# Banus/pano360

Hardware: AMD Instinct MI355X
Metric: blended megapixels/sec (multiband) (higher is better)
Workload: dtype f32; 1 GPU; cfg3: 32 synthetic 3840x2160 frames per image set, spherical warp + multiband blend L=5, native resolution (MAX_RESOLUTION uncapped); frames=32

## Files before the change

### include/pano360.h

```cpp
#ifndef PANO360_H
#define PANO360_H

#include <stddef.h>
#include <stdint.h>

#ifdef __cplusplus
extern "C" {
#endif

#define PANO_OK 0
#define PANO_EINVAL (-1)
#define PANO_EHIP (-2)
#define PANO_ELIMIT (-3)
#define PANO_ESOLVE (-4)

#define PANO_MAX_TAPS 129
#define PANO_MAX_LEVELS 8
#define PANO_TAP_LEAD 7
#define PANO_TAP_PAD 40
#ifndef PANO_INTERIOR_BLOCK
#define PANO_INTERIOR_BLOCK 4
#endif
#ifndef PANO_MEDIAN_KEEP
#define PANO_MEDIAN_KEEP 32
// ... 46 lines not shown


const char *pano_version(void);
const char *pano_last_error(void);
int pano_device_count(void);
int pano_pitch(int w);
int pano_interior_block(void);

typedef struct pano_ctx pano_ctx;
#define PANO_OPT_BLUR_KERNEL 0
#define PANO_OPT_OWN_PRUNE 1
#define PANO_OPT_BLUR_SEGMENTS 2
#define PANO_OPT_BLUR_LEAN 3
#define PANO_OPT_STITCH_STREAMS 4
#define PANO_OPT_STITCH_ASYNC 5
#define PANO_OPT_BLUR_SEG_LEN 6
#define PANO_OPT_SIFT_GRAPH 7
#define PANO_OPT_LEVEL_CLASSES 8
#define PANO_OPT_COUNT 9
#define PANO_BLUR_MFMA 0
#define PANO_BLUR_VALU 1
int pano_ctx_create(int device, void *stream, pano_ctx **out);
int pano_ctx_destroy(pano_ctx *ctx);
int pano_ctx_set_stream(pano_ctx *ctx, void *stream);
int pano_ctx_set_option(pano_ctx *ctx, int option, int value);
int pano_ctx_get_option(const pano_ctx *ctx, int option, int *value);

int pano_timing_enable(pano_ctx *ctx, int on);
int pano_kernel_count(void);
const char *pano_kernel_name(int kid);
int pano_timing_read(pano_ctx *ctx, int kid, double *total_ms, int *launches);

int pano_add_weights(pano_ctx *ctx, const uint8_t *frame, int h, int w,
                     const float *lut255, const double *hat_x, const double *hat_y,
                     float *rgba);

int pano_warp_spherical(pano_ctx *ctx, const uint8_t *frame, int sh, int sw,
                        const double *proj, const double *sin_t, const double *cos_t,
                        const double *tan_p, const float *lut255, const double *hat_x,
                        const double *hat_y, int gx0, int gy0, int pw, int ph,
                        float *planes, uint8_t *mask, float *map_x, float *map_y);

int pano_warp_windows(pano_ctx *ctx, const pano_camera *cams, const pano_patch *patches,
                      int n, int max_vw, int max_vh, const double *sin_t,
                      const double *cos_t, const double *tan_p, const float *lut,
                      int lut_stride, const uint8_t *need);

int pano_ownership(pano_ctx *ctx, const pano_patch *patches, int n, int H, int W,
                   int16_t *owner, uint8_t *valid);

int pano_ownership_cameras(pano_ctx *ctx, const pano_camera *cams, int n, int H, int W,
                           int xs0, int xs1, const double *sin_t, const double *cos_t,
                           const double *tan_p, int16_t *owner, uint8_t *valid);

int pano_owned_regions(pano_ctx *ctx, const int16_t *owner, int H, int W, int xs0, int xs1,
                       int n, int min_gap, int max_spans, uint8_t *marks,
                       int32_t *regions);

int pano_ownership_regions(pano_ctx *ctx, const pano_camera *cams, int n, int H, int W,
                           int xs0, int xs1, const double *sin_t, const double *cos_t,
                           const double *tan_p, int16_t *owner, uint8_t *valid,
                           int min_gap, int max_spans, uint8_t *marks, int32_t *regions);

int pano_blur_tile_grid(const pano_ctx *ctx);
int pano_blur_tiles(pano_ctx *ctx, const pano_patch *patches, int n, int max_aw,
                    int max_ah, int W, int radius, const uint8_t *interior,
                    uint8_t *tile_flags, uint8_t *warp_need);
int pano_multiband_blur_prepare(pano_ctx *ctx, const pano_patch *patches, int n,
                                int max_aw, int max_ah, int W, const uint8_t *interior,
                                uint8_t *tile_flags);
int pano_multiband_blur(pano_ctx *ctx, const pano_patch *patches, int n, int max_aw,
                        int max_vh, int max_ah, const int16_t *owner, int W,
                        const float *taps, const int *ntaps, int n_blur,
                        const uint8_t *interior, uint8_t *tile_flags);

int pano_interior_map(pano_ctx *ctx, const int16_t *owner, int H, int W, int xs0, int xs1,
                      int radius, int16_t *block_owner, uint8_t *interior);
int pano_interior_classes(pano_ctx *ctx, const int16_t *owner, int H, int W, int xs0, int xs1,
                          const int *radii, int n_radii, int16_t *block_owner, uint8_t *interior,
                          uint8_t *classes);

int pano_layout_windows(int tile_grid, const int32_t *regions, int n, int max_spans,
                        const int32_t *rects, const uint8_t *have, int radius,
                        int xs0, int xs1, int n_blur, pano_patch *records, int cap,
                        pano_layout *out);
int pano_layout_place(pano_patch *records, int n_records, void *planes, void *blurred,
                      void *scratch);

int pano_multiband_compose(pano_ctx *ctx, const pano_patch *patches, int n, int H, int W,
                           int xs0, int xs1, int n_levels, const int16_t *owner,
                           const uint8_t *valid, const uint8_t *interior,
                           const uint8_t *classes, const pano_camera *cams,
                           const double *sin_t, const double *cos_t, const double *tan_p,
                           const float *lut, int lut_stride, uint8_t *mosaic,
                           float *mosaic_f32);

int pano_blend_cameras(pano_ctx *ctx, const pano_camera *cams, int n, int H, int W,
                       int xs0, int xs1, int linear, const double *sin_t,
                       const double *cos_t, const double *tan_p, const float *lut,
                       int lut_stride, uint8_t *mosaic, uint8_t *valid);

int pano_median_cameras(pano_ctx *ctx, const pano_camera *cams, int n, int H, int W,
                        int xs0, int xs1, float tol, const double *sin_t,
                        const double *cos_t, const double *tan_p, const float *lut,
                        int lut_stride, uint8_t *mosaic, uint8_t *valid);

// ... 321 lines not shown
```

### pano360_amd/_lib.py

```python
import ctypes as C
import os
import subprocess

_HERE = os.path.dirname(os.path.abspath(__file__))
LIB_PATH = os.environ.get("PANO_LIB") or os.path.join(_HERE, "libpano360_hip.so")

MAX_TAPS = 129
MAX_LEVELS = 8
TAP_LEAD = 7
TAP_PAD = 40
OPT_BLUR_KERNEL, OPT_OWN_PRUNE, OPT_BLUR_SEGMENTS, OPT_BLUR_LEAN, OPT_STITCH_STREAMS = 0, 1, 2, 3, 4
OPT_STITCH_ASYNC = 5
OPT_BLUR_SEG_LEN = 6
OPT_SIFT_GRAPH = 7
OPT_LEVEL_CLASSES = 8
BLUR_MFMA, BLUR_VALU = 0, 1


class PanoError(RuntimeError):
    """A C-ABI call returned a negative status."""


class Patch(C.Structure):
    _fields_ = [("planes", C.c_void_p), ("mask", C.c_void_p),
# ... 86 lines not shown
class PhotoFrame(C.Structure):
    _fields_ = [("img", C.c_void_p), ("pitch", C.c_int64), ("w", C.c_int32), ("h", C.c_int32)]


class PhotoPair(C.Structure):
    _fields_ = [("H", C.c_double * 9), ("i", C.c_int32), ("j", C.c_int32)]


class PhotoApply(C.Structure):
    _fields_ = [("src", C.c_void_p), ("dst", C.c_void_p), ("table", C.c_void_p),
                ("src_pitch", C.c_int64), ("dst_pitch", C.c_int64),
                ("w", C.c_int32), ("h", C.c_int32)]


class Pair(C.Structure):
    _fields_ = [("minv", C.c_double * 9), ("i", C.c_int32), ("j", C.c_int32)]


class SiftKeypoint(C.Structure):
    _fields_ = [("x", C.c_float), ("y", C.c_float), ("size", C.c_float), ("angle", C.c_float),
                ("response", C.c_float), ("octave", C.c_int32), ("r", C.c_int32), ("c", C.c_int32)]


class Camera(C.Structure):
    _fields_ = [("proj", C.c_double * 9), ("frame", C.c_void_p),
                ("hat_x", C.c_void_p), ("hat_y", C.c_void_p),
                ("sh", C.c_int32), ("sw", C.c_int32),
                ("y0", C.c_int32), ("x0", C.c_int32), ("h", C.c_int32), ("w", C.c_int32)]


_vp, _i = C.c_void_p, C.c_int
_SIGNATURES = {
    "pano_version": (C.c_char_p, []),
    "pano_last_error": (C.c_char_p, []),
    "pano_device_count": (_i, []),
    "pano_pitch": (_i, [_i]),
    "pano_interior_block": (_i, []),
    "pano_ctx_create": (_i, [_i, _vp, C.POINTER(C.c_void_p)]),
    "pano_ctx_destroy": (_i, [_vp]),
    "pano_ctx_set_stream": (_i, [_vp, _vp]),
    "pano_ctx_set_option": (_i, [_vp, _i, _i]),
    "pano_ctx_get_option": (_i, [_vp, _i, C.POINTER(C.c_int)]),
    "pano_timing_enable": (_i, [_vp, _i]),
    "pano_kernel_count": (_i, []),
    "pano_kernel_name": (C.c_char_p, [_i]),
    "pano_timing_read": (_i, [_vp, _i, C.POINTER(C.c_double), C.POINTER(C.c_int)]),
    "pano_add_weights": (_i, [_vp, _vp, _i, _i, _vp, _vp, _vp, _vp]),
    "pano_warp_spherical": (_i, [_vp, _vp, _i, _i, _vp, _vp, _vp, _vp, _vp, _vp, _vp, _i, _i, _i,
                                 _i, _vp, _vp, _vp, _vp]),
    "pano_warp_windows": (_i, [_vp, _vp, _vp, _i, _i, _i, _vp, _vp, _vp, _vp, _i, _vp]),
    "pano_blur_tiles": (_i, [_vp, _vp, _i, _i, _i, _i, _i, _vp, _vp, _vp]),
    "pano_ownership": (_i, [_vp, _vp, _i, _i, _i, _vp, _vp]),
    "pano_ownership_cameras": (_i, [_vp, _vp, _i, _i, _i, _i, _i, _vp, _vp, _vp, _vp, _vp]),
    "pano_owned_regions": (_i, [_vp, _vp, _i, _i, _i, _i, _i, _i, _i, _vp, _vp]),
    "pano_ownership_regions": (_i, [_vp, _vp, _i, _i, _i, _i, _i, _vp, _vp, _vp, _vp, _vp,
                                    _i, _i, _vp, _vp]),
    "pano_multiband_blur": (_i, [_vp, _vp, _i, _i, _i, _i, _vp, _i, _vp, C.POINTER(C.c_int), _i,
                                 _vp, _vp]),
    "pano_multiband_blur_prepare": (_i, [_vp, _vp, _i, _i, _i, _i, _vp, _vp]),
    "pano_layout_windows": (_i, [_i, _vp, _i, _i, _vp, _vp, _i, _i, _i, _i, _vp, _i, _vp]),
    "pano_layout_place": (_i, [_vp, _i, _vp, _vp, _vp]),
    "pano_interior_map": (_i, [_vp, _vp, _i, _i, _i, _i, _i, _vp, _vp]),
    "pano_interior_classes": (_i, [_vp, _vp, _i, _i, _i, _i, _vp, _i, _vp, _vp, _vp]),
    "pano_multiband_compose": (_i, [_vp, _vp, _i, _i, _i, _i, _i, _i, _vp, _vp, _vp, _vp, _vp, _vp,
                                    _vp, _vp, _vp, _i, _vp, _vp]),
    "pano_blend_cameras": (_i, [_vp, _vp, _i, _i, _i, _i, _i, _i, _vp, _vp, _vp, _vp, _i, _vp,
                                _vp]),
    "pano_blur_tile_grid": (_i, [_vp]),
    "pano_overlap_blocks": (_i, [_i, _i]),
    "pano_overlap_stats": (_i, [_vp, _vp, _vp, _i, _i, _i, _i, _vp, _vp, _vp]),
    "pano_linear_blend": (_i, [_vp, _vp, _i, _i, _i, _vp]),
    "pano_no_blend": (_i, [_vp, _vp, _i, _i, _i, _vp]),
    "pano_median_cameras": (_i, [_vp, _vp, _i, _i, _i, _i, _i, C.c_float, _vp, _vp, _vp, _vp, _i,
                                 _vp, _vp]),
    "pano_median_blend": (_i, [_vp, _vp, _i, _i, _i, C.c_float, _vp]),
    "pano_crop_rect": (_i, [_vp, _vp, _i, _i, _vp, _vp]),
    "pano_blur_plane": (_i, [_vp, _vp, _vp, _vp, _i, _i, _i, _vp, _i]),
    "pano_pyr_down": (_i, [_vp, _vp, _i, _i, _vp]),
    "pano_gray_u8": (_i, [_vp, _vp, _i, _i, _vp]),
    "pano_scale_step": (_i, [_vp, _vp, _i, _i, _vp, _i, _vp, _vp]),
    "pano_scale_space": (_i, [_vp, _vp, _i, _i, _i, _i, _vp, _vp, _vp, _vp, _vp]),
    "pano_resize_up2": (_i, [_vp, _vp, _i, _i, _vp]),
    "pano_decimate2": (_i, [_vp, _vp, _i, _i, _vp]),
    "pano_subtract": (_i, [_vp, _vp, _vp, C.c_size_t, _vp]),
    "pano_pyr_down_image": (_i, [_vp, _vp, _i, _i, _i, _i, _vp]),
    "pano_pyr_up_image": (_i, [_vp, _vp, _i, _i, _i, _i, _vp, _i, _vp, _i, _i]),
    "pano_u8_to_f32": (_i, [_vp, _vp, C.c_size_t, _vp]),
    "pano_laplacian_mix": (_i, [_vp, _vp, _vp, _vp, C.c_size_t, _i, _vp]),
    "pano_clip_u8": (_i, [_vp, _vp, C.c_size_t, _i, _vp]),
    "pano_poisson_blend": (_i, [_vp, _vp, _vp, _vp, _i, _i, _i, C.c_double, _i, _vp, _vp, _vp]),
    "pano_seam_levels": (_i, [_vp, _vp, _vp, _i, _i, _i, _i, _i, _vp, _vp]),
    "pano_seam_flood": (_i, [_vp, _vp, _i, _i, _i, _i, _vp, _vp]),
    "pano_seam_mask": (_i, [_vp, _vp, _i, _i, _vp, _vp, _vp, _i, _i]),
    "pano_alpha_blend": (_i, [_vp, _vp, _vp, _i, _vp, _i, C.c_int64, C.c_int64, C.c_int64, _i, _i,
                              _i, _vp]),
    "pano_resize_u8": (_i, [_vp, _vp, _i, _i, _i, _vp, _vp, _vp, _i, _i]),
    "pano_sift_extrema": (_i, [_vp, _vp, _i, _i, _i, _i, C.c_float, C.c_float, C.c_float, _vp,
                               _vp, _i]),
    "pano_sift_orient": (_i, [_vp, _vp, _vp, _i, _vp, _vp, _i, _vp, _vp, _i]),
    "pano_sift_describe": (_i, [_vp, _vp, _vp, _i, _vp, _i, _vp, _vp]),
    "pano_sift_sort_work_bytes": (C.c_size_t, [_i]),
    "pano_sift_sort_unique": (_i, [_vp, _vp, _i, _vp, _i, _vp, _vp, _vp]),
    "pano_knn2_work_bytes": (C.c_size_t, [_i, _i, _i]),
    "pano_knn2": (_i, [_vp, _vp, _i, _vp, _i, _i, C.c_float, _vp, _vp, _vp, _vp]),
    "pano_hom_ransac_work_bytes": (C.c_size_t, [_i, _i]),
    "pano_hom_ransac": (_i, [_vp, _vp, _vp, _vp, _i, _i, C.c_float, C.c_uint64, _vp, _vp, _vp, _vp,
# ... 134 lines not shown
```

### pano360_amd/csrc/blend.hip

```cpp
#include <stdlib.h>

#include "geom.h"

__global__ __launch_bounds__(256) void ownership_kernel(
    const pano_patch *__restrict__ patches, int n, int H, int W,
    int16_t *__restrict__ owner, uint8_t *__restrict__ valid) {
    const int x = blockIdx.x * 64 + threadIdx.x, y = blockIdx.y * 4 + threadIdx.y;
    if (x >= W || y >= H) return;
    float best = 0.0f;
    int who = -1;
    bool any = false;
    for (int i = 0; i < n; ++i) {
        const pano_patch p = patches[i];
        const int px = x - p.x0, py = y - p.y0;
        if ((unsigned)px >= (unsigned)p.w || (unsigned)py >= (unsigned)p.h) continue;
        const float a = p.planes[3 * (size_t)p.vh * p.vpitch + (size_t)py * p.vpitch + px];
        if (a > best) {
            best = a;
            who = i;
        }
        any |= p.mask[(size_t)py * p.w + px] == 0;
    }
    owner[(size_t)y * W + x] = (int16_t)who;
    valid[(size_t)y * W + x] = any ? 1 : 0;
// ... 355 lines not shown
#pragma unroll 1
        for (int y = sy0 + wave; y < sy1; y += 4) {
            const double t = tan_p[y];
            float best = 0.0f;
            int who = -1, who_k = 0;
            bool any = false;
            for (int k = 0; k < ncand; ++k) {
                const int i = listed < 0 ? k : __builtin_amdgcn_readfirstlane(list[k]);
                const pano_camera *cam = cams + i;
                const int px = xc - cam->x0, py = y - cam->y0;
                if ((unsigned)px >= (unsigned)cam->w || (unsigned)py >= (unsigned)cam->h) continue;
                float fx, fy;
                const int sw = cam->sw, sh_ = cam->sh;
                if (map_pixel(cam->proj, s, c, t, sw, sh_, fx, fy)) continue;
                any = true;
                const Taps tp = make_taps_unmasked(fx, fy, sw, sh_);
                const float a = alpha_at(cam->hat_x, cam->hat_y, tp);
                if (a > best) {
                    best = a;
                    who = i;
                    who_k = k;
                }
            }
            if (in_strip) {
                owner[(size_t)y * W + x] = (int16_t)who;
                valid[(size_t)y * W + x] = any ? 1 : 0;
            }
            if (marks) {
                if (who != run_o) {
                    flush();
                    run_o = who;
                    run_pos = pruned && who >= 0 ? s_pos[sub][who_k] : who_k;
                    run_y0 = y;
                }
                run_y1 = y;
            }
        }
    }
    if (!marks) return;
    flush();
    __syncthreads();
    const int tid = wave * 64 + lane;
    if (tid < listed) {
        const int *b = s_box[tid];
        if (b[1] >= b[0]) box_merge(boxes + (size_t)box_stride * sh.list[tid], b[0], b[1], b[2], b[3]);
    }
}

#define OW_T 64
#define OW_Q 16
#define OW_CAMS 32
#define OW_QLIST 8
#define OW_ILP 4
#define OW_EVAL (-3)
#define OW_NOBODY (-1)
#define OW_UNOWNED (-2)

#define OW_SUBS 8
#define OW_FN(name) name
#include "own_tile.inc"
#undef OW_FN
#define OW_TH_TALL (OW_Q * OW_SUBS)

template <bool LINEAR, bool PERCAM>
__global__ __launch_bounds__(256) void blend_cameras_kernel(
    const pano_camera *__restrict__ cams, int n, int H, int W, int xs0, int xs1,
    const double *__restrict__ sin_t, const double *__restrict__ cos_t,
    const double *__restrict__ tan_p, const float *__restrict__ lut,
    uint8_t *__restrict__ mosaic, uint8_t *__restrict__ valid) {
    __shared__ CamList sh;
    __shared__ CamPrune pr;
    __shared__ float s_lut[256];
    if (!PERCAM) s_lut[threadIdx.y * 64 + threadIdx.x] = lut[threadIdx.y * 64 + threadIdx.x];
    const int bx0 = xs0 + blockIdx.x * 64, by0 = blockIdx.y * 4;
    const int bx1 = min(bx0 + 64, xs1), by1 = min(by0 + 4, H);
    const int listed = build_camera_list(sh, cams, n, bx0, bx1, by0, by1);
    const Candidates cand = prune_masked_cameras(pr, sh, listed, cams, n, bx0, bx1, by0, by1,
                                                 sin_t, cos_t, tan_p);

    const int x = bx0 + threadIdx.x, y = by0 + threadIdx.y;
    if (x >= xs1 || y >= H) return;
    const double s = sin_t[x], c = cos_t[x], t = tan_p[y];
    float acc[3] = {0.0f, 0.0f, 0.0f}, wsum = 0.0f;
    uint8_t last[3] = {0, 0, 0};
    bool any = false;
    for (int kk = 0; kk < cand.count; ++kk) {
        const int k = LINEAR ? kk : cand.count - 1 - kk;
        const int i = cand.list ? __builtin_amdgcn_readfirstlane(cand.list[k]) : k;
        const pano_camera *cam = cams + i;
        float fx, fy, rgb[3];
        if (!camera_sees(cam, x, y, s, c, t, fx, fy)) continue;
        any = true;
        const Taps tp = sample_camera(cam, PERCAM ? lut + (size_t)i * 256 : s_lut, fx, fy, rgb);
        if (LINEAR) {
            const float a = alpha_at(cam->hat_x, cam->hat_y, tp);
#pragma unroll
            for (int ch = 0; ch < 3; ++ch) acc[ch] = acc[ch] + rgb[ch] * a;
            wsum = wsum + a;
        } else {
#pragma unroll
            for (int ch = 0; ch < 3; ++ch) last[ch] = (uint8_t)(int)(255.0f * rgb[ch]);
            break;
        }
    }
    const size_t g = ((size_t)y * W + x) * 3;
    if (LINEAR) {
// ... 583 lines not shown
extern "C" int pano_owned_regions(pano_ctx *ctx, const int16_t *owner, int H, int W, int xs0,
                                  int xs1, int n, int min_gap, int max_spans, uint8_t *marks,
                                  int32_t *regions) {
    PANO_ENTER(ctx, "pano_owned_regions");
    PANO_REQUIRE(owner && marks && regions, "pano_owned_regions: null pointer");
    PANO_REQUIRE(H > 0 && W > 0 && n >= 0 && n <= 32767 && max_spans >= 1 && min_gap >= 0,
                 "pano_owned_regions: bad argument");
    if (int rc = check_strip(xs0, xs1, W, "pano_owned_regions")) return rc;
    if (n == 0) return PANO_OK;
    hipStream_t s = (hipStream_t)stream;
    const int stride = 5 + 2 * max_spans;
    if (int rc = launch_init_regions(s, regions, n, stride, marks, W)) return rc;
    if (xs0 == xs1) return PANO_OK;
    dim3 block(64, 4), grid(ceil_div(xs1 - xs0, 512), ceil_div(H, 4));
    PANO_TIMED(PK_OWNED_BOXES, s,
               hipLaunchKernelGGL(owned_boxes_kernel, grid, block, 0, s, owner, H, W, xs0, xs1,
                                  regions, stride, marks));
    PANO_LAUNCH_CHECK("owned_boxes_kernel");
    PANO_TIMED(PK_OWNED_SPANS, s,
               hipLaunchKernelGGL(owned_spans_kernel, dim3(n), dim3(256), 0, s, marks, W, xs0, xs1,
                                  min_gap, max_spans, stride, regions));
    PANO_LAUNCH_CHECK("owned_spans_kernel");
    return PANO_OK;
}

extern "C" int pano_ownership_regions(pano_ctx *ctx, const pano_camera *cams, int n, int H, int W,
                                      int xs0, int xs1, const double *sin_t, const double *cos_t,
                                      const double *tan_p, int16_t *owner, uint8_t *valid,
                                      int min_gap, int max_spans, uint8_t *marks,
                                      int32_t *regions) {
    PANO_ENTER(ctx, "pano_ownership_regions");
    if (int rc = check_table(cams, n, H, W, "pano_ownership_regions")) return rc;
    PANO_REQUIRE(sin_t && cos_t && tan_p && owner && valid && marks && regions,
                 "pano_ownership_regions: null pointer");
    if (int rc = check_strip(xs0, xs1, W, "pano_ownership_regions")) return rc;
    PANO_REQUIRE(max_spans >= 1 && min_gap >= 0, "pano_ownership_regions: bad argument");
    if (n == 0) return PANO_OK;
    hipStream_t s = (hipStream_t)stream;
    const int stride = 5 + 2 * max_spans;
    if (int rc = launch_init_regions(s, regions, n, stride, marks, W)) return rc;
    if (xs0 == xs1) return PANO_OK;
    const int prune = ctx->opt[PANO_OPT_OWN_PRUNE];
    dim3 block(64, 4), grid(ceil_div(xs1 - xs0, 64), ceil_div(H, (prune & 2) ? OWN_TILE_ROWS : OW_TH_TALL));
    PANO_TIMED(PK_OWNERSHIP_CAMS, s,
               hipLaunchKernelGGL((prune & 2) ? ownership_cameras_l1_kernel : ownership_cameras_kernel,
                                  grid, block, (prune & 2) ? 0 : own_shared_bytes(n), s, cams, n, H, W, xs0,
                                  xs1, sin_t, cos_t, tan_p, owner, valid, prune & 1, regions, stride,
                                  marks));
    PANO_LAUNCH_CHECK("ownership_cameras_kernel");
    PANO_TIMED(PK_OWNED_SPANS, s,
               hipLaunchKernelGGL(owned_spans_kernel, dim3(n), dim3(256), 0, s, marks, W, xs0, xs1,
                                  min_gap, max_spans, stride, regions));
    PANO_LAUNCH_CHECK("owned_spans_kernel");
    return PANO_OK;
}

static int interior_map_launch(pano_ctx *ctx, const int16_t *owner, int H, int W, int xs0, int xs1,
                               const int *radii, int n_radii, int16_t *block_owner,
                               uint8_t *interior, uint8_t *classes, const char *who) {
    void *const stream = (void *)ctx->stream;
    PANO_REQUIRE(owner && block_owner && interior && radii, "%s: null pointer", who);
    PANO_REQUIRE(H > 0 && W > 0 && n_radii >= 1 && n_radii < PANO_MAX_LEVELS, "%s: bad argument", who);
    if (int rc = check_strip(xs0, xs1, W, who)) return rc;
    LevelReaches lv = {};
    lv.n = n_radii;
    for (int k = 0; k < n_radii; ++k) {
        PANO_REQUIRE(radii[k] >= 0 && (k == 0 || radii[k] >= radii[k - 1]),
                     "%s: radii must ascend (level %d: %d)", who, k, radii[k]);
        lv.reach[k] = ceil_div(radii[k] + IB - 1, IB);
    }
    const int radius = radii[n_radii - 1];
    const int H8 = ceil_div(H, IB), W8 = ceil_div(W, IB), reach = lv.reach[n_radii - 1];
    if (xs0 == xs1) return PANO_OK;
    const int ilo = xs0 / IB, ihi = ceil_div(xs1, IB);
    const int blo = ilo - reach > 0 ? ilo - reach : 0, bhi = ihi + reach < W8 ? ihi + reach : W8;
    dim3 block(64, 4), grid(ceil_div(bhi - blo, 64), ceil_div(H8, 4));
    hipStream_t s = (hipStream_t)stream;
    PANO_TIMED(PK_INTERIOR, s,
               hipLaunchKernelGGL(block_owner_kernel, grid, block, 0, s, owner, H, W, xs0, xs1,
                                  H8, W8, blo, bhi, block_owner));
    PANO_LAUNCH_CHECK("block_owner_kernel");
    PANO_REQUIRE(reach <= IT_REACH_MAX, "%s: radius %d reaches %d blocks (at most %d)", who, radius,
                 reach, IT_REACH_MAX);
    hipLaunchKernelGGL(interior_tile_kernel, dim3(ceil_div(ihi - ilo, IT_W), ceil_div(H8, IT_H)),
                       dim3(256), 0, s, block_owner, H8, W8, reach, blo, bhi, ilo, ihi, interior, lv,
                       classes);
    PANO_LAUNCH_CHECK("interior_tile_kernel");
    return PANO_OK;
}

extern "C" int pano_interior_map(pano_ctx *ctx, const int16_t *owner, int H, int W, int xs0,
                                 int xs1, int radius, int16_t *block_owner, uint8_t *interior) {
    PANO_ENTER(ctx, "pano_interior_map");
    return interior_map_launch(ctx, owner, H, W, xs0, xs1, &radius, 1, block_owner, interior, nullptr,
                               "pano_interior_map");
}

extern "C" int pano_interior_classes(pano_ctx *ctx, const int16_t *owner, int H, int W, int xs0,
                                     int xs1, const int *radii, int n_radii, int16_t *block_owner,
                                     uint8_t *interior, uint8_t *classes) {
    PANO_ENTER(ctx, "pano_interior_classes");
    PANO_REQUIRE(classes, "pano_interior_classes: null pointer");
    return interior_map_launch(ctx, owner, H, W, xs0, xs1, radii, n_radii, block_owner, interior,
                               classes, "pano_interior_classes");
}

// ... 179 lines not shown
```

### pano360_amd/csrc/geom.h

```cpp
#pragma once
#include "common.h"

struct Taps {
    int x0, x1, y0, y1;
    float w00, w01, w10, w11;
};

__device__ __forceinline__ Taps tap_base(float px, float py) {
    int sx = cv_round(px * 32.0f), sy = cv_round(py * 32.0f);
    int fx = sx & 31, fy = sy & 31;
    Taps t;
    t.x0 = sat16(sx >> 5);
    t.y0 = sat16(sy >> 5);
    t.x1 = t.x0 + 1;
    t.y1 = t.y0 + 1;
    float ax = (float)fx * (1.0f / 32.0f), ay = (float)fy * (1.0f / 32.0f);
    t.w00 = (1.0f - ay) * (1.0f - ax);
    t.w01 = (1.0f - ay) * ax;
    t.w10 = ay * (1.0f - ax);
    t.w11 = ay * ax;
    return t;
}

__device__ __forceinline__ void reflect_taps(Taps &t, int sw, int sh) {
    t.x1 = reflect_edge(t.x0 + 1, sw);
    t.x0 = reflect_edge(t.x0, sw);
    t.y1 = reflect_edge(t.y0 + 1, sh);
    t.y0 = reflect_edge(t.y0, sh);
}

__device__ __forceinline__ Taps make_taps(float px, float py, int sw, int sh) {
    Taps t = tap_base(px, py);
    reflect_taps(t, sw, sh);
    return t;
}

__device__ __forceinline__ bool taps_interior(const Taps &t, int sw, int sh) {
    return (unsigned)t.x0 < (unsigned)(sw - 1) && (unsigned)t.y0 < (unsigned)(sh - 1);
}

__device__ __forceinline__ Taps make_taps_unmasked(float px, float py, int sw, int sh) {
    Taps t = tap_base(px, py);
    t.x1 = min(t.x1, sw - 1);
    t.y1 = min(t.y1, sh - 1);
    return t;
}

__device__ __forceinline__ float lerp4(float v00, float v01, float v10, float v11,
                                       const Taps &t) {
    float a = v00 * t.w00;
    a = a + v01 * t.w01;
    a = a + v10 * t.w10;
    a = a + v11 * t.w11;
    return a;
}

struct TapBytes {
    uint32_t v[4][3];
};
typedef uint32_t u32_any __attribute__((aligned(1)));
typedef uint16_t u16_any __attribute__((aligned(1)));
typedef const __attribute__((address_space(1))) uint8_t *frame_ptr;
typedef const __attribute__((address_space(1))) u32_any *frame_ptr32;
typedef const __attribute__((address_space(1))) u16_any *frame_ptr16;

#define PANO_BYTE_X4(B)                                                                        \
    __device__ __forceinline__ uint32_t byte##B##_x4(uint32_t x) {                             \
        uint32_t r;                                                                            \
        asm("v_lshlrev_b32_sdwa %0, %1, %2 dst_sel:DWORD dst_unused:UNUSED_PAD "               \
            "src0_sel:DWORD src1_sel:BYTE_" #B                                                 \
            : "=v"(r)                                                                          \
            : "v"(2u), "v"(x));                                                                \
        return r;                                                                              \
    }
// ... 145 lines not shown
```

### pano360_amd/csrc/own_tile.inc

```
#define OW_TH (OW_Q * OW_SUBS)
#define OW_NQ (4 * OW_SUBS)

struct OW_FN(OwnShared) {
    CamList cl;
    pano_camera cam[OW_CAMS];
    double sn[OW_T], cs[OW_T], tn[OW_TH];
    double rq[4][4];
    double rall[4];
    double step2;
    double rsub[OW_SUBS][2];
    int low1[OW_SUBS], ncand[OW_SUBS];
    int subfill[OW_SUBS];
    float hi2[OW_NQ][OW_QLIST];
    int low2[OW_NQ];
    short qlist[OW_NQ][OW_QLIST];
    int qn[OW_NQ];
    int qfill[OW_NQ];
    int evalq[OW_NQ], n_eval;
    alignas(16) short town[OW_TH][OW_T];
};
static inline size_t OW_FN(own_shared_bytes)(int n) {
    const size_t nl = (size_t)(n < OWN_LIST ? n : OWN_LIST);
    return sizeof(OW_FN(OwnShared)) + nl * (16 + 4 * OW_SUBS + 2 * OW_SUBS) + 16;
}

template <int MODE>
__device__ __forceinline__ void OW_FN(own_tile)(OW_FN(OwnShared) &S, int (*__restrict__ s_box)[4],
                                         float *__restrict__ s_hi, short *__restrict__ s_keep, int NL,
                                         const pano_camera *__restrict__ cams, int n,
                                         int H, int W, int bx0, int bx1, int by0, int by1,
                                         int listed, int prune, int vt, int16_t *__restrict__ owner,
                                         uint8_t *__restrict__ valid, int32_t *__restrict__ boxes,
                                         int box_stride, uint8_t *__restrict__ marks) {
    const int lane = threadIdx.x, wave = threadIdx.y, tid = wave * 64 + lane;
    auto index_at = [&](int pos) -> int { return listed < 0 ? pos : S.cl.list[pos]; };
    auto cam_at = [&](int pos) -> const pano_camera * {
        if (MODE == 1) return &S.cam[pos];
        if (MODE == 2) return &S.cam[index_at(pos)];
        return cams + index_at(pos);
    };

    if (listed == 0) {
        if (tid < OW_NQ) S.qfill[tid] = OW_NOBODY;
        __syncthreads();
    } else if (prune && listed > 0) {
        for (int t = vt; t < OW_SUBS * listed; t += 256) {
            const int sub = t / listed, k = t - sub * listed;
            const int sy0 = by0 + OW_Q * sub, sy1 = min(sy0 + OW_Q, H);
            float hi = -1.0f;
            if (sy0 < H) {
                const double rng[6] = {S.rall[0], S.rall[1], S.rsub[sub][0], S.rsub[sub][1],
                                       S.rall[2], S.rall[3]};
                const pano_camera *cam = cam_at(k);
                const int cb_ = bx1 - 1 - bx0;
                const double sa = S.sn[0], ca = S.cs[0], sb = S.sn[cb_], cb = S.cs[cb_];
                const bool narrow = (double)(cb_ * cb_) * S.step2 <= 0.0625;
                const AlphaBound bnd = narrow ? alpha_bound_ends(cam, sa, ca, sb, cb, S.rsub[sub][0], S.rsub[sub][1])
                                              : alpha_bound(cam, rng);
                hi = bnd.hi;
                if (bnd.lo > 0.0f && tile_inside(cam, bx0, bx1, sy0, sy1))
                    atomicMax(&S.low1[sub], __float_as_int(bnd.lo));
            }
            s_hi[sub * NL + k] = hi;
        }
        __syncthreads();
        for (int sub = wave; sub < OW_SUBS; sub += 4) {
            const float L = __int_as_float(S.low1[sub]);
            int nc = 0;
            for (int base = 0; base < listed; base += 64) {
                const int k = base + lane;
                const bool keep = k < listed && s_hi[sub * NL + k] >= L;
                const unsigned long long bal = __ballot(keep);
                if (keep) s_keep[sub * NL + nc + __popcll(bal & ((1ull << lane) - 1ull))] = (short)k;
                nc += __popcll(bal);
            }
            if (lane == 0) {
                S.ncand[sub] = nc;
                int whole = -1;
                if (nc == 1 && L > 0.0f) {
                    const int pos = s_keep[sub * NL];
                    const int sy0 = by0 + OW_Q * sub, sy1 = min(sy0 + OW_Q, H);
                    if (tile_inside(cam_at(pos), bx0, bx1, sy0, sy1)) whole = index_at(pos);
                }
                S.subfill[sub] = whole;
            }
        }
        __syncthreads();
// ... 24 lines not shown
                                              : alpha_bound(cam, rng);
                hi = bnd.hi;
                if (bnd.lo > 0.0f && tile_inside(cam, qx0, qx1, sy0, sy1))
                    atomicMax(&S.low2[sub * 4 + q], __float_as_int(bnd.lo));
            }
            S.hi2[sub * 4 + q][j] = hi;
        }
        __syncthreads();
        if (tid < OW_NQ) {
            const int sub = tid >> 2, q = tid & 3, nc = S.ncand[sub];
            const int sy0 = by0 + OW_Q * sub, sy1 = min(sy0 + OW_Q, H);
            const int qx0 = bx0 + OW_Q * q, qx1 = min(qx0 + OW_Q, bx1);
            int fill = OW_EVAL, qn = -1;
            if (sy0 >= H || qx0 >= bx1 || nc == 0) {
                fill = OW_NOBODY;
            } else if (S.subfill[sub] >= 0) {
                fill = S.subfill[sub];
            } else if (nc <= OW_QLIST) {
                const float L = __int_as_float(S.low2[tid]);
                qn = 0;
                for (int j = 0; j < nc; ++j)
                    if (S.hi2[tid][j] >= L) S.qlist[tid][qn++] = s_keep[sub * NL + j];
                if (qn == 0) {
                    fill = OW_NOBODY;
                } else if (qn == 1 && L > 0.0f) {
                    const int pos = S.qlist[tid][0];
                    if (tile_inside(cam_at(pos), qx0, qx1, sy0, sy1)) fill = index_at(pos);
                }
            }
            S.qn[tid] = qn;
            S.qfill[tid] = fill;
        }
        __syncthreads();
    }
    if (wave == 0) {
        static_assert(OW_NQ <= 64, "one ballot lists the quarters to evaluate");
        const bool e = lane < OW_NQ && S.qfill[lane] == OW_EVAL && by0 + OW_Q * (lane >> 2) < H &&
                       bx0 + OW_Q * (lane & 3) < bx1;
        const unsigned long long bal = __ballot(e);
        if (e) S.evalq[__popcll(bal & ((1ull << lane) - 1ull))] = lane;
        if (lane == 0) S.n_eval = __popcll(bal);
    }
    __syncthreads();
    constexpr int PER_Q = 4 / OW_ILP;
    const int n_items = PER_Q * S.n_eval;
#pragma unroll 1
    for (int item = wave; item < n_items; item += 4) {
        const int qid = S.evalq[item / PER_Q], sub = qid >> 2, q = qid & 3;
        const int col = OW_Q * q + (lane & (OW_Q - 1));
        const int row0 = OW_Q * sub + 4 * OW_ILP * (item % PER_Q) + (lane >> 4);
        const int xc = min(bx0 + col, bx1 - 1);
        const double s = S.sn[col], c = S.cs[col];
        double t[OW_ILP];
        int y[OW_ILP], who[OW_ILP];
        float best[OW_ILP];
        bool any[OW_ILP];
#pragma unroll
        for (int j = 0; j < OW_ILP; ++j) {
            t[j] = S.tn[row0 + 4 * j];
            y[j] = min(by0 + row0 + 4 * j, by1 - 1);
            best[j] = 0.0f;
            who[j] = -1;
            any[j] = false;
        }
        const int mode = S.qn[qid];
        const int ncand = mode >= 0 ? mode : (mode == -1 ? S.ncand[sub] : (listed < 0 ? n : listed));
        for (int k = 0; k < ncand; ++k) {
            const int pos = __builtin_amdgcn_readfirstlane(
                mode >= 0 ? (int)S.qlist[qid][k] : (mode == -1 ? (int)s_keep[sub * NL + k] : k));
            const pano_camera *cam = cam_at(pos);
            const int i = index_at(pos);
            const int px = xc - cam->x0, sw = cam->sw, sh_ = cam->sh;
            const int cam_y0 = cam->y0, cam_h = cam->h;
            const bool in_x = (unsigned)px < (unsigned)cam->w;
            Taps tp[OW_ILP];
            bool ok[OW_ILP];
#pragma unroll
            for (int j = 0; j < OW_ILP; ++j) {
                float fx, fy;
                const bool m = map_pixel(cam->proj, s, c, t[j], sw, sh_, fx, fy);
                ok[j] = in_x & ((unsigned)(y[j] - cam_y0) < (unsigned)cam_h) & !m;
                tp[j] = make_taps_unmasked(ok[j] ? fx : 0.0f, ok[j] ? fy : 0.0f, sw, sh_);
            }
            typedef const __attribute__((address_space(1))) double *hat_ptr;
            const hat_ptr hat_x = (hat_ptr)cam->hat_x, hat_y = (hat_ptr)cam->hat_y;
            double hx0[OW_ILP], hx1[OW_ILP], hy0[OW_ILP], hy1[OW_ILP];
#pragma unroll
            for (int j = 0; j < OW_ILP; ++j) {
                hy0[j] = hat_y[tp[j].y0];
                hy1[j] = hat_y[tp[j].y1];
                hx0[j] = hat_x[tp[j].x0];
                hx1[j] = hat_x[tp[j].x1];
            }
#pragma unroll
            for (int j = 0; j < OW_ILP; ++j) {
                const float a = lerp4((float)(hy0[j] * hx0[j]), (float)(hy0[j] * hx1[j]),
                                      (float)(hy1[j] * hx0[j]), (float)(hy1[j] * hx1[j]), tp[j]);
                any[j] |= ok[j];
                const bool wins = ok[j] & (a > best[j]);
                best[j] = wins ? a : best[j];
                who[j] = wins ? i : who[j];
            }
        }
#pragma unroll
        for (int j = 0; j < OW_ILP; ++j)
            S.town[row0 + 4 * j][col] = (short)(who[j] >= 0 ? who[j] : (any[j] ? OW_UNOWNED : OW_NOBODY));
    }
    __syncthreads();
    const int rows = by1 - by0, ncols = min(bx1 - bx0, OW_T);
    typedef short short8 __attribute__((ext_vector_type(8)));
    typedef short8 short8_any __attribute__((aligned(2)));
    typedef unsigned int uint2v __attribute__((ext_vector_type(2)));
    typedef uint2v uint2_any __attribute__((aligned(1)));
#pragma unroll
    for (int k = 0; k < OW_TH / 32; ++k) {
        const int row = 32 * k + 8 * wave + (lane >> 3), c0 = 8 * (lane & 7);
        if (row >= rows || c0 >= ncols) continue;
        const int fill = S.qfill[(row >> 4) * 4 + (c0 >> 4)];
        short8 w8 = (short)fill;
        if (fill == OW_EVAL) w8 = *(const short8 *)&S.town[row][c0];
        short8 own8;
        unsigned char ok8[8];
#pragma unroll
        for (int j = 0; j < 8; ++j) {
            const int w = w8[j];
            own8[j] = (short)(w < 0 ? -1 : w);
            ok8[j] = (w >= 0 || w == OW_UNOWNED) ? 1 : 0;
        }
        const size_t g = (size_t)(by0 + row) * W + bx0 + c0;
        if (c0 + 8 <= ncols) {
            *(short8_any *)(owner + g) = own8;
            uint2v v;
            v.x = ok8[0] | ok8[1] << 8 | ok8[2] << 16 | (unsigned)ok8[3] << 24;
            v.y = ok8[4] | ok8[5] << 8 | ok8[6] << 16 | (unsigned)ok8[7] << 24;
            *(uint2_any *)(valid + g) = v;
        } else {
            for (int j = 0; j < ncols - c0; ++j) {
                owner[g + j] = own8[j];
                valid[g + j] = ok8[j];
            }
        }
    }
    if (!marks) return;
    const int x = bx0 + lane;
    const bool in_strip = x < bx1;
    auto flush = [&](int run_o, int run_y0, int run_y1) {
        if (run_o < 0 || !in_strip) return;
        marks[(size_t)run_o * W + x] = 1;
        if (n <= OWN_LIST) {
            int *b = s_box[run_o];
            atomicMin(&b[0], run_y0);
            atomicMax(&b[1], run_y1);
            atomicMin(&b[2], x);
            atomicMax(&b[3], x);
        } else {
            box_merge(boxes + (size_t)box_stride * run_o, run_y0, run_y1, x, x);
        }
    };
#pragma unroll 1
    for (int sub = wave; sub < OW_SUBS; sub += 4) {
        const int r0 = OW_Q * sub, r1 = min(r0 + OW_Q, rows);
        if (r0 >= rows) break;
        const int fill = S.qfill[sub * 4 + (lane >> 4)];
        if (fill != OW_EVAL) {
            if (fill >= 0 && in_strip) {
                marks[(size_t)fill * W + x] = 1;
                if ((lane & 15) == 0) {
                    const int x1 = min(x + OW_Q, bx1) - 1;
                    if (n <= OWN_LIST) {
                        int *b = s_box[fill];
                        atomicMin(&b[0], by0 + r0);
                        atomicMax(&b[1], by0 + r1 - 1);
                        atomicMin(&b[2], x);
                        atomicMax(&b[3], x1);
                    } else {
                        box_merge(boxes + (size_t)box_stride * fill, by0 + r0, by0 + r1 - 1, x, x1);
                    }
                }
            }
        } else {
            int run_o = -1, run_y0 = 0, run_y1 = 0;
            for (int row = r0; row < r1; ++row) {
                const int t = S.town[row][lane], w = t < 0 ? -1 : t;
                const int y = by0 + row;
                if (w != run_o) {
                    flush(run_o, run_y0, run_y1);
                    run_o = w;
                    run_y0 = y;
                }
                run_y1 = y;
            }
            flush(run_o, run_y0, run_y1);
        }
    }
    __syncthreads();
    if (n <= OWN_LIST && tid < n) {
        const int *b = s_box[tid];
        if (b[1] >= b[0]) box_merge(boxes + (size_t)box_stride * tid, b[0], b[1], b[2], b[3]);
    }
}

__global__ __launch_bounds__(256) void OW_FN(ownership_cameras_kernel)(
    const pano_camera *__restrict__ cams, int n, int H, int W, int xs0, int xs1,
    const double *__restrict__ sin_t, const double *__restrict__ cos_t,
    const double *__restrict__ tan_p, int16_t *__restrict__ owner,
    uint8_t *__restrict__ valid, int prune, int32_t *__restrict__ boxes, int box_stride,
    uint8_t *__restrict__ marks) {
    extern __shared__ __align__(16) unsigned char own_smem[];
    OW_FN(OwnShared) &S = *(OW_FN(OwnShared) *)own_smem;
    const int NL = min(n, OWN_LIST);
    int (*s_box)[4] = (int (*)[4])(own_smem + ((sizeof(OW_FN(OwnShared)) + 15) & ~(size_t)15));
    float *s_hi = (float *)(s_box + NL);
    short *s_keep = (short *)(s_hi + OW_SUBS * NL);
    const int lane = threadIdx.x, wave = threadIdx.y, tid = wave * 64 + lane;
    const int bx0 = xs0 + blockIdx.x * OW_T, by0 = blockIdx.y * OW_TH;
    const int bx1 = min(bx0 + OW_T, xs1), by1 = min(by0 + OW_TH, H);
    const int vt = (tid + 64 * (int)((blockIdx.x + blockIdx.y) & 3)) & 255;
    if (marks && tid < NL) {
        int *b = s_box[tid];
        b[0] = b[2] = 0x7fffffff;
        b[1] = b[3] = -1;
    }
    constexpr int DW = (int)(sizeof(pano_camera) / 4);
    const bool all_cams = n <= OW_CAMS;
    uint32_t rec_dw[(OW_CAMS * DW + 255) / 256];
    if (all_cams) {
#pragma unroll
        for (int r = 0; r < (OW_CAMS * DW + 255) / 256; ++r) {
            const int d = tid + 256 * r;
            rec_dw[r] = d < n * DW ? ((const uint32_t *)cams)[d] : 0u;
        }
    }
    double tv = 0.0, tw = 0.0;
    if (wave == 0) {
        const int xc = min(bx0 + lane, bx1 - 1);
        tv = table_f64(sin_t, xc);
        tw = table_f64(cos_t, xc);
    }
    double trow[OW_TH / 64 > 0 ? OW_TH / 64 : 1];
    if (wave == 1) {
#pragma unroll
        for (int r = 0; r < OW_TH / 64; ++r) trow[r] = table_f64(tan_p, min(by0 + 64 * r + lane, by1 - 1));
    }
    const int listed = build_camera_list(S.cl, cams, n, bx0, bx1, by0, by1);
    const int mode = all_cams ? 2 : (listed >= 0 && listed <= OW_CAMS ? 1 : 0);
    uint32_t *dst = (uint32_t *)S.cam;
    if (all_cams) {
#pragma unroll
        for (int r = 0; r < (OW_CAMS * DW + 255) / 256; ++r) {
            const int d = tid + 256 * r;
            if (d < n * DW) dst[d] = rec_dw[r];
        }
    } else if (mode == 1) {
        for (int d = tid; d < listed * DW; d += 256) {
            const int rec = d / DW, w = d - rec * DW;
            dst[d] = ((const uint32_t *)(cams + S.cl.list[rec]))[w];
        }
    }
    if (wave == 0) {
        S.sn[lane] = tv;
        S.cs[lane] = tw;
        double lo_s = tv, hi_s = tv, lo_c = tw, hi_c = tw;
#pragma unroll
        for (int off = 1; off < 64; off <<= 1) {
            lo_s = fmin(lo_s, __shfl_xor(lo_s, off, 64));
            hi_s = fmax(hi_s, __shfl_xor(hi_s, off, 64));
            lo_c = fmin(lo_c, __shfl_xor(lo_c, off, 64));
// ... 46 lines not shown
```

### pano360_amd/csrc/warp.hip

```cpp
#include "geom.h"

struct ProjK {
    double p[9];
};

template <bool FULL>
__global__ __launch_bounds__(256) void warp_spherical_kernel(
    const uint8_t *__restrict__ frame, int sh, int sw, ProjK K,
    const double *__restrict__ sin_t, const double *__restrict__ cos_t,
    const double *__restrict__ tan_p, const float *__restrict__ lut255,
    const double *__restrict__ hat_x, const double *__restrict__ hat_y,
    int gx0, int gy0, int pw, int ph, int pitch, float *__restrict__ planes,
    uint8_t *__restrict__ mask, float *__restrict__ map_x,
    float *__restrict__ map_y) {
    __shared__ float s_lut[256];
    s_lut[threadIdx.y * 64 + threadIdx.x] = lut255[threadIdx.y * 64 + threadIdx.x];
    __syncthreads();

    const int x = blockIdx.x * 64 + threadIdx.x;
    const int y = blockIdx.y * 4 + threadIdx.y;
    if (x >= pw || y >= ph) return;

    float px, py;
    const bool m = map_pixel(K.p, sin_t[gx0 + x], cos_t[gx0 + x], tan_p[gy0 + y], sw, sh,
// ... 125 lines not shown
                                  frame, h, w, lut255, hat_x, hat_y, (float4 *)rgba));
    PANO_LAUNCH_CHECK("add_weights_kernel");
    return PANO_OK;
}

static int check_frame(const char *who, int sh, int sw, int pw, int ph, int gx0, int gy0) {
    PANO_REQUIRE(sh > 0 && sw > 0 && sh < 32767 && sw < 32767,
                 "%s: frame %dx%d outside (0, 32767)", who, sh, sw);
    PANO_REQUIRE(pw > 0 && ph > 0 && gx0 >= 0 && gy0 >= 0, "%s: bad rectangle", who);
    return PANO_OK;
}

extern "C" int pano_warp_spherical(pano_ctx *ctx, const uint8_t *frame, int sh, int sw,
                                   const double *proj, const double *sin_t, const double *cos_t,
                                   const double *tan_p, const float *lut255, const double *hat_x,
                                   const double *hat_y, int gx0, int gy0, int pw, int ph,
                                   float *planes, uint8_t *mask, float *map_x, float *map_y) {
    PANO_ENTER(ctx, "pano_warp_spherical");
    PANO_REQUIRE(frame && proj && sin_t && cos_t && tan_p && lut255 && hat_x &&
                     hat_y && planes && mask,
                 "pano_warp_spherical: null pointer");
    PANO_REQUIRE((map_x == nullptr) == (map_y == nullptr),
                 "pano_warp_spherical: map_x and map_y must both be given or both be NULL");
    if (int rc = check_frame("pano_warp_spherical", sh, sw, pw, ph, gx0, gy0)) return rc;
    ProjK K;
    for (int i = 0; i < 9; ++i) K.p[i] = proj[i];
    dim3 block(64, 4), grid(ceil_div(pw, 64), ceil_div(ph, 4));
    PANO_TIMED(PK_WARP, (hipStream_t)stream,
               hipLaunchKernelGGL(warp_spherical_kernel<true>, grid, block, 0,
                                  (hipStream_t)stream, frame, sh, sw, K, sin_t, cos_t, tan_p,
                                  lut255, hat_x, hat_y, gx0, gy0, pw, ph, pano_pitch_of(pw),
                                  planes, mask, map_x, map_y));
    PANO_LAUNCH_CHECK("warp_spherical_kernel");
    return PANO_OK;
}

extern "C" int pano_warp_windows(pano_ctx *ctx, const pano_camera *cams, const pano_patch *patches,
                                 int n, int max_vw, int max_vh, const double *sin_t,
                                 const double *cos_t, const double *tan_p, const float *lut,
                                 int lut_stride, const uint8_t *need) {
    PANO_ENTER(ctx, "pano_warp_windows");
    PANO_REQUIRE(cams && patches && sin_t && cos_t && tan_p && lut && lut_stride >= 0,
                 "pano_warp_windows: null pointer");
    PANO_REQUIRE(n >= 0 && n <= 65535 && max_vw >= 0 && max_vh >= 0,
                 "pano_warp_windows: bad argument");
    if (n == 0 || max_vw == 0 || max_vh == 0) return PANO_OK;
    dim3 block(64, 4), grid(ceil_div(max_vw, 64), ceil_div(max_vh, 4 * WARP_ROWS), n);
    PANO_TIMED(PK_WARP_WINDOWS, (hipStream_t)stream,
               hipLaunchKernelGGL(warp_windows_kernel, grid, block, 0, (hipStream_t)stream,
                                  cams, patches, sin_t, cos_t, tan_p, lut, lut_stride, need));
    PANO_LAUNCH_CHECK("warp_windows_kernel");
    return PANO_OK;
}
```

Baseline: 204,000 MP/s.

## Raise ownership kernel occupancy via LDS union, scalarized camera loads, deferred taps

The ownership-cameras kernel gets a launch-bounds occupancy hint, and its shared struct overlaps the hi2 scratch with the tile owner buffer in a union to shrink LDS. Per-camera fields (projection matrix, hat pointers, sizes) are forced uniform with readfirstlane so they live in scalar registers. Tap computation is split so only fixed-point coordinates stay live across the hat-table loads, and the hat loads go through table_f64. Residency query entry points are added for inspecting occupancy. The register cap risks spills, and the union is only safe if hi2 and town are never live at the same time.

```diff
diff --git a/include/pano360.h b/include/pano360.h
--- a/include/pano360.h
+++ b/include/pano360.h
@@ -122,6 +122,9 @@
 int pano_ownership_cameras(pano_ctx *ctx, const pano_camera *cams, int n, int H, int W,
                            int xs0, int xs1, const double *sin_t, const double *cos_t,
                            const double *tan_p, int16_t *owner, uint8_t *valid);
+
+int pano_ownership_residency(int n, int *blocks_per_cu, int *lds_bytes);
+int pano_warp_windows_residency(int *blocks_per_cu);
 
 int pano_owned_regions(pano_ctx *ctx, const int16_t *owner, int H, int W, int xs0, int xs1,
                        int n, int min_gap, int max_spans, uint8_t *marks,
diff --git a/pano360_amd/_lib.py b/pano360_amd/_lib.py
--- a/pano360_amd/_lib.py
+++ b/pano360_amd/_lib.py
@@ -162,6 +162,8 @@
     "pano_blur_tiles": (_i, [_vp, _vp, _i, _i, _i, _i, _i, _vp, _vp, _vp]),
     "pano_ownership": (_i, [_vp, _vp, _i, _i, _i, _vp, _vp]),
     "pano_ownership_cameras": (_i, [_vp, _vp, _i, _i, _i, _i, _i, _vp, _vp, _vp, _vp, _vp]),
+    "pano_ownership_residency": (_i, [_i, C.POINTER(C.c_int), C.POINTER(C.c_int)]),
+    "pano_warp_windows_residency": (_i, [C.POINTER(C.c_int)]),
     "pano_owned_regions": (_i, [_vp, _vp, _i, _i, _i, _i, _i, _i, _i, _vp, _vp]),
     "pano_ownership_regions": (_i, [_vp, _vp, _i, _i, _i, _i, _i, _vp, _vp, _vp, _vp, _vp,
                                     _i, _i, _vp, _vp]),
diff --git a/pano360_amd/csrc/blend.hip b/pano360_amd/csrc/blend.hip
--- a/pano360_amd/csrc/blend.hip
+++ b/pano360_amd/csrc/blend.hip
@@ -431,6 +431,7 @@
 #define OW_CAMS 32
 #define OW_QLIST 8
 #define OW_ILP 4
+#define OW_WAVES 6
 #define OW_EVAL (-3)
 #define OW_NOBODY (-1)
 #define OW_UNOWNED (-2)
@@ -1120,6 +1121,14 @@
                hipLaunchKernelGGL(owned_spans_kernel, dim3(n), dim3(256), 0, s, marks, W, xs0, xs1,
                                   min_gap, max_spans, stride, regions));
     PANO_LAUNCH_CHECK("owned_spans_kernel");
+    return PANO_OK;
+}
+
+extern "C" int pano_ownership_residency(int n, int *blocks_per_cu, int *lds_bytes) {
+    PANO_REQUIRE(n >= 0 && blocks_per_cu && lds_bytes, "pano_ownership_residency: bad argument");
+    *lds_bytes = (int)own_shared_bytes(n);
+    PANO_HIP(hipOccupancyMaxActiveBlocksPerMultiprocessor(blocks_per_cu, ownership_cameras_kernel, 256,
+                                                          own_shared_bytes(n)));
     return PANO_OK;
 }
 
diff --git a/pano360_amd/csrc/geom.h b/pano360_amd/csrc/geom.h
--- a/pano360_amd/csrc/geom.h
+++ b/pano360_amd/csrc/geom.h
@@ -6,8 +6,9 @@
     float w00, w01, w10, w11;
 };
 
-__device__ __forceinline__ Taps tap_base(float px, float py) {
-    int sx = cv_round(px * 32.0f), sy = cv_round(py * 32.0f);
+__device__ __forceinline__ int tap_fixed(float p) { return cv_round(p * 32.0f); }
+
+__device__ __forceinline__ Taps tap_base_fixed(int sx, int sy) {
     int fx = sx & 31, fy = sy & 31;
     Taps t;
     t.x0 = sat16(sx >> 5);
@@ -20,6 +21,10 @@
     t.w10 = ay * (1.0f - ax);
     t.w11 = ay * ax;
     return t;
+}
+
+__device__ __forceinline__ Taps tap_base(float px, float py) {
+    return tap_base_fixed(tap_fixed(px), tap_fixed(py));
 }
 
 __device__ __forceinline__ void reflect_taps(Taps &t, int sw, int sh) {
diff --git a/pano360_amd/csrc/own_tile.inc b/pano360_amd/csrc/own_tile.inc
--- a/pano360_amd/csrc/own_tile.inc
+++ b/pano360_amd/csrc/own_tile.inc
@@ -11,13 +11,15 @@
     double rsub[OW_SUBS][2];
     int low1[OW_SUBS], ncand[OW_SUBS];
     int subfill[OW_SUBS];
-    float hi2[OW_NQ][OW_QLIST];
     int low2[OW_NQ];
     short qlist[OW_NQ][OW_QLIST];
     int qn[OW_NQ];
     int qfill[OW_NQ];
     int evalq[OW_NQ], n_eval;
-    alignas(16) short town[OW_TH][OW_T];
+    union {
+        alignas(16) short town[OW_TH][OW_T];
+        float hi2[OW_NQ][OW_QLIST];
+    };
 };
 static inline size_t OW_FN(own_shared_bytes)(int n) {
     const size_t nl = (size_t)(n < OWN_LIST ? n : OWN_LIST);
@@ -32,7 +34,7 @@
                                          int listed, int prune, int vt, int16_t *__restrict__ owner,
                                          uint8_t *__restrict__ valid, int32_t *__restrict__ boxes,
                                          int box_stride, uint8_t *__restrict__ marks) {
-    const int lane = threadIdx.x, wave = threadIdx.y, tid = wave * 64 + lane;
+    const int lane = threadIdx.x, wave = __builtin_amdgcn_readfirstlane(threadIdx.y), tid = wave * 64 + lane;
     auto index_at = [&](int pos) -> int { return listed < 0 ? pos : S.cl.list[pos]; };
     auto cam_at = [&](int pos) -> const pano_camera * {
         if (MODE == 1) return &S.cam[pos];
@@ -163,13 +165,12 @@
         const int xc = min(bx0 + col, bx1 - 1);
         const double s = S.sn[col], c = S.cs[col];
         double t[OW_ILP];
-        int y[OW_ILP], who[OW_ILP];
+        int who[OW_ILP];
         float best[OW_ILP];
         bool any[OW_ILP];
 #pragma unroll
         for (int j = 0; j < OW_ILP; ++j) {
             t[j] = S.tn[row0 + 4 * j];
-            y[j] = min(by0 + row0 + 4 * j, by1 - 1);
             best[j] = 0.0f;
             who[j] = -1;
             any[j] = false;
@@ -181,32 +182,46 @@
                 mode >= 0 ? (int)S.qlist[qid][k] : (mode == -1 ? (int)s_keep[sub * NL + k] : k));
             const pano_camera *cam = cam_at(pos);
             const int i = index_at(pos);
-            const int px = xc - cam->x0, sw = cam->sw, sh_ = cam->sh;
-            const int cam_y0 = cam->y0, cam_h = cam->h;
-            const bool in_x = (unsigned)px < (unsigned)cam->w;
-            Taps tp[OW_ILP];
+            auto uni = [](int v) { return __builtin_amdgcn_readfirstlane(v); };
+            auto uni64 = [&](unsigned long long b) {
+                const unsigned lo = (unsigned)uni((int)(unsigned)b), hi = (unsigned)uni((int)(unsigned)(b >> 32));
+                return ((unsigned long long)hi << 32) | lo;
+            };
+            double K[9];
+#pragma unroll
+            for (int e = 0; e < 9; ++e)
+                K[e] = __longlong_as_double((long long)uni64((unsigned long long)__double_as_longlong(cam->proj[e])));
+            const double *hat_x = (const double *)uni64((unsigned long long)cam->hat_x);
+            const double *hat_y = (const double *)uni64((unsigned long long)cam->hat_y);
+            const int sw = uni(cam->sw), sh_ = uni(cam->sh);
+            const int cam_y0 = uni(cam->y0), cam_h = uni(cam->h);
+            const bool in_x = (unsigned)(xc - uni(cam->x0)) < (unsigned)uni(cam->w);
+            int yb = by0 + row0;
+            asm volatile("" : "+v"(yb));
+            int sx[OW_ILP], sy[OW_ILP];
             bool ok[OW_ILP];
 #pragma unroll
             for (int j = 0; j < OW_ILP; ++j) {
                 float fx, fy;
-                const bool m = map_pixel(cam->proj, s, c, t[j], sw, sh_, fx, fy);
-                ok[j] = in_x & ((unsigned)(y[j] - cam_y0) < (unsigned)cam_h) & !m;
-                tp[j] = make_taps_unmasked(ok[j] ? fx : 0.0f, ok[j] ? fy : 0.0f, sw, sh_);
-            }
-            typedef const __attribute__((address_space(1))) double *hat_ptr;
-            const hat_ptr hat_x = (hat_ptr)cam->hat_x, hat_y = (hat_ptr)cam->hat_y;
+                const bool m = map_pixel(K, s, c, t[j], sw, sh_, fx, fy);
+                ok[j] = in_x & ((unsigned)(min(yb + 4 * j, by1 - 1) - cam_y0) < (unsigned)cam_h) & !m;
+                sx[j] = tap_fixed(ok[j] ? fx : 0.0f);
+                sy[j] = tap_fixed(ok[j] ? fy : 0.0f);
+            }
             double hx0[OW_ILP], hx1[OW_ILP], hy0[OW_ILP], hy1[OW_ILP];
 #pragma unroll
             for (int j = 0; j < OW_ILP; ++j) {
-                hy0[j] = hat_y[tp[j].y0];
-                hy1[j] = hat_y[tp[j].y1];
-                hx0[j] = hat_x[tp[j].x0];
-                hx1[j] = hat_x[tp[j].x1];
+                const int x0 = sat16(sx[j] >> 5), y0 = sat16(sy[j] >> 5);
+                hy0[j] = table_f64(hat_y, y0);
+                hy1[j] = table_f64(hat_y, min(y0 + 1, sh_ - 1));
+                hx0[j] = table_f64(hat_x, x0);
+                hx1[j] = table_f64(hat_x, min(x0 + 1, sw - 1));
             }
 #pragma unroll
             for (int j = 0; j < OW_ILP; ++j) {
+                const Taps tp = tap_base_fixed(sx[j], sy[j]);
                 const float a = lerp4((float)(hy0[j] * hx0[j]), (float)(hy0[j] * hx1[j]),
-                                      (float)(hy1[j] * hx0[j]), (float)(hy1[j] * hx1[j]), tp[j]);
+                                      (float)(hy1[j] * hx0[j]), (float)(hy1[j] * hx1[j]), tp);
                 any[j] |= ok[j];
                 const bool wins = ok[j] & (a > best[j]);
                 best[j] = wins ? a : best[j];
@@ -311,7 +326,7 @@
     }
 }
 
-__global__ __launch_bounds__(256) void OW_FN(ownership_cameras_kernel)(
+__global__ __launch_bounds__(256, OW_WAVES) void OW_FN(ownership_cameras_kernel)(
     const pano_camera *__restrict__ cams, int n, int H, int W, int xs0, int xs1,
     const double *__restrict__ sin_t, const double *__restrict__ cos_t,
     const double *__restrict__ tan_p, int16_t *__restrict__ owner,
@@ -323,7 +338,7 @@
     int (*s_box)[4] = (int (*)[4])(own_smem + ((sizeof(OW_FN(OwnShared)) + 15) & ~(size_t)15));
     float *s_hi = (float *)(s_box + NL);
     short *s_keep = (short *)(s_hi + OW_SUBS * NL);
-    const int lane = threadIdx.x, wave = threadIdx.y, tid = wave * 64 + lane;
+    const int lane = threadIdx.x, wave = __builtin_amdgcn_readfirstlane(threadIdx.y), tid = wave * 64 + lane;
     const int bx0 = xs0 + blockIdx.x * OW_T, by0 = blockIdx.y * OW_TH;
     const int bx1 = min(bx0 + OW_T, xs1), by1 = min(by0 + OW_TH, H);
     const int vt = (tid + 64 * (int)((blockIdx.x + blockIdx.y) & 3)) & 255;
diff --git a/pano360_amd/csrc/warp.hip b/pano360_amd/csrc/warp.hip
--- a/pano360_amd/csrc/warp.hip
+++ b/pano360_amd/csrc/warp.hip
@@ -201,3 +201,9 @@
     PANO_LAUNCH_CHECK("warp_windows_kernel");
     return PANO_OK;
 }
+
+extern "C" int pano_warp_windows_residency(int *blocks_per_cu) {
+    PANO_REQUIRE(blocks_per_cu, "pano_warp_windows_residency: null pointer");
+    PANO_HIP(hipOccupancyMaxActiveBlocksPerMultiprocessor(blocks_per_cu, warp_windows_kernel, 256, 0));
+    return PANO_OK;
+}
```

After: 206,000 MP/s (median of 3 runs). Within noise of the previous version (+1.0%).
